# mscaudill/openseize

Hardware: AMD Instinct MI355X
Metric: Msamples/sec/node (FIR+IIR chain, 256ch f64); HBM GB/s vs roofline at 1/2/4/8 GPU (higher is better)
Workload: dtype f64

## Files before the change

openseize_amd/csrc/chain_spec.hip:

```cpp
#include <algorithm>
#include <cmath>
#include <functional>
#include <vector>

#include "common.h"
#include "fft4096.h"
#include "fir_pair.h"
#include "handles.h"
#include "sos_tile.h"
#include "chain_spec.h"
#include "chain_zp.h"

namespace osz {

struct SpecArgs {
    FirArgs f;
    int64_t n;
    int64_t W;
    int nruns;
    int la, lb;
    int R;
    const double *M;
    const double *P;
    const double *Lrow;
// ... 425 lines not shown
    hipLaunchKernelGGL(spec_poison_kernel, dim3((nch + 255) / 256), dim3(256), 0, st, s->dcarry[s->cur],
                       4095 + 256 * s->R, sos->dstate, sos->nsec, nch);
    OSZ_HIP(hipGetLastError());
    s->true_valid = true;
    return OSZ_OK;
}

int spec_touch(ChainSpec *s, hipStream_t st) {
    if (!s) return OSZ_OK;
    int rc = spec_settle(s, st);
    if (rc) return rc;
    s->carry_valid = false;
    return OSZ_OK;
}

using spec_kern_t = void (*)(SpecArgs);
template <int NM, int HP>
static spec_kern_t spec_kernel_for(int nr) {
    static const spec_kern_t k[8] = {
        chain_spec_kernel<8, NM, HP>,  chain_spec_kernel<9, NM, HP>,  chain_spec_kernel<10, NM, HP>,
        chain_spec_kernel<11, NM, HP>, chain_spec_kernel<12, NM, HP>, chain_spec_kernel<13, NM, HP>,
        chain_spec_kernel<14, NM, HP>, chain_spec_kernel<15, NM, HP>};
    return k[nr - 8];
}

static int specn_forward(ChainSpec *s, const double *x, int64_t ldx, int64_t n, double *f, int64_t ldf,
                         hipStream_t st, const std::function<int()> &between, bool *taken) {
    osz_fir_s *fir = s->fir;
    const int NB = s->NR, S = 256 * NB;
    if (n < 2 * (int64_t)S) return OSZ_OK;
    if (!s->carry_valid) {
        int rc = spec_import(s, st);
        if (rc) return rc;
    }
    {
        int rc = between();
        if (rc) return rc;
    }
    const int64_t W = (n - 1) / S;
    int64_t nruns = 512 / fir->nch;
    if (nruns > W) nruns = W;
    if (nruns < 1) nruns = 1;
    ZpArgs g{};
    g.f.x = x;
    g.f.y = f;
    g.f.ldx = ldx;
    g.f.ldy = ldf;
    g.f.n = n;
    g.f.skip = 0;
    g.f.wlen = fir->ntaps;
    g.f.step = S;
    g.f.H = s->dH;
    g.f.tb = fir->tb;
    g.n = n;
    g.W = W;
    g.nruns = (int)nruns;
    g.la = (int)(n - W * S);
    g.R = s->R;
    g.Rf = s->R;
    g.nh = s->nh;
    g.Lrow = s->dT;
    g.carry_in = s->dcarry[s->cur];
    g.carry_out = s->dcarry[s->cur ^ 1];
    if (n >= s->hist_cap) {
        g.hist = s->dhist[s->hcur];
        g.hist_len = s->hist_cap;
        s->hist_n = s->hist_cap;
    } else {
        const int64_t keep = std::min<int64_t>(s->hist_n, s->hist_cap - n);
        double *dst = s->dhist[s->hcur ^ 1];
        if (keep > 0)
            OSZ_HIP(hipMemcpy2DAsync(dst, sizeof(double) * s->hist_cap,
                                     s->dhist[s->hcur] + (s->hist_n - keep), sizeof(double) * s->hist_cap,
                                     sizeof(double) * keep, fir->nch, hipMemcpyDeviceToDevice, st));
        OSZ_HIP(hipMemcpy2DAsync(dst + keep, sizeof(double) * s->hist_cap, x, sizeof(double) * ldx,
                                 sizeof(double) * n, fir->nch, hipMemcpyDeviceToDevice, st));
        s->hcur ^= 1;
        s->hist_n = keep + n;
    }
    s->since_import += n;
    zp_kern_t kern = zpn_fwd_kernel_for(NB, s->NM, s->NS);
    if (!kern) return fail(OSZ_ERR_STATE, "forward chain kernel: no instance for %d rows, %d modes (%d slow)", NB, s->NM, s->NS);
    const int ns = 2 * s->nh;
    const size_t lds = sizeof(fft::cube::C2) * fft::cube::SLOTS +
                       sizeof(double) * (ns + 2 * s->R * s->NS * 2 + s->NM * 2 + 20 * s->NM * 2 + 2 * s->NS * ns) + 1024;
    OSZ_DYN_LDS(kern, lds);
    {
        KernelTimer kt("chain_fwd", st);
        hipLaunchKernelGGL(kern, dim3((unsigned)nruns, fir->nch), dim3(256), lds, st, g);
    }
    OSZ_HIP(hipGetLastError());
    {
        int rcs = sos_seal_launch(g.f.y, g.f.ldy, n, (int)nruns, W, nruns, (int64_t)S, nullptr, 0, fir->nch,
                                  g.carry_out, kSpecLdc, kSpecLdc, st);
        if (rcs) return rcs;
    }
    s->cur ^= 1;
    s->true_valid = false;
    *taken = true;
    return OSZ_OK;
}


static int spec_link(osz_fir_s *fir, osz_sos_s *sos, hipStream_t st, ChainSpec **out) {
    ChainSpec *s = sos->spec;
    if (s && s->fir != fir) {
        int rc = spec_settle(s, st);
        if (rc) return rc;
        spec_unlink(s);
        s = nullptr;
    }
    if (!s && fir->spec) {
        int rc = spec_settle(fir->spec, st);
        if (rc) return rc;
        spec_unlink(fir->spec);
    }
    if (!s) {
        s = new ChainSpec();
        s->fir = fir;
        s->sos = sos;
        fir->spec = sos->spec = s;
        int rc = spec_build(s);
        if (rc) {
            spec_unlink(s);
            return rc;
        }
    }
    *out = s;
    return OSZ_OK;
}

static spec_kern_t spec_kernel_pick(const ChainSpec *s) {
    if (s->NR < 8 || s->NR > 15) return nullptr;
    return s->NM == 2 ? spec_kernel_for<2, 16>(s->NR) : s->NM == 4 ? spec_kernel_for<4, 16>(s->NR)
           : s->NM == 6 ? spec_kernel_for<6, 16>(s->NR) : nullptr;
}

int spec_route(osz_fir_s *fir, osz_sos_s *sos, hipStream_t st, int *route) {
    ChainSpec *s = nullptr;
    int rc = spec_link(fir, sos, st, &s);
    if (rc) return rc;
    *route = !s->eligible ? 0 : s->nega ? 2 : 1;
    return OSZ_OK;
}

int spec_plan(osz_fir_s *fir, osz_sos_s *sos, hipStream_t st, int *route, int *rows, int *nm, int *ns,
              int *has) {
    int rc = spec_route(fir, sos, st, route);
    if (rc || *route == 0) return rc;
    const ChainSpec *s = sos->spec;
    *rows = s->NR;
    *nm = s->NM;
    *ns = s->nega ? s->NS : 0;
    *has = (s->nega ? zpn_fwd_kernel_for(s->NR, s->NM, s->NS) != nullptr : spec_kernel_pick(s) != nullptr);
    return OSZ_OK;
}

int spec_try_forward(osz_fir_s *fir, osz_sos_s *sos, const double *x, int64_t ldx, int64_t n, double *f,
                     int64_t ldf, hipStream_t st, const std::function<int()> &between, bool *taken) {
    *taken = false;
    ChainSpec *s = nullptr;
    {
        int rc = spec_link(fir, sos, st, &s);
        if (rc) return rc;
    }
    if (!s->eligible) return OSZ_OK;
    if (s->nega) return specn_forward(s, x, ldx, n, f, ldf, st, between, taken);
    const int NR = s->NR, S = 256 * NR;
// ... 81 lines not shown
```

openseize_amd/csrc/chain_zp.h:

```cpp
#pragma once

#include "chain_spec.h"
#include "fft4096.h"
#include "fir_pair.h"
#include "handles.h"
#include "nega_window.h"

namespace osz {

struct ZpArgs {
    FirArgs f;
    double *y0;
    int64_t ldy0, n0;
    int64_t n;
    int64_t W;
    int nruns;
    int la, lb;
    int R, Rf, nh;
    const double *M;
    const double *P;
    const double *Lrow;
    const double *carry_in;
    double *carry_out;
    const double *held_in;
    double *held_out;
    double *hist;
    int hist_len;
    long long *nanpos;
    long long pos;
    int wclose;
};

__host__ __device__ __forceinline__ int64_t zp_run_start(int64_t r, int64_t W, int nruns, int wclose) {
    if (r <= 0) return 0;
    if (r >= nruns) return W;
    if (W < 8 * (int64_t)nruns) return (r * W) / nruns;
    const int64_t V = W + (nruns - 1) + wclose;
    const int64_t s = (r * V) / nruns - (r - 1);
    return s < W - (nruns - r) ? s : W - (nruns - r);
}

template <int NM>
__device__ __forceinline__ void zp_powers(const double *ptab, int e, double *pr, double *pi) {
    const double *p1 = ptab + ((e >> 5) * NM) * 2, *p2 = ptab + ((8 + ((e >> 2) & 7)) * NM) * 2,
                 *p3 = ptab + ((16 + (e & 3)) * NM) * 2;
#pragma unroll
    for (int q = 0; q < NM; ++q) {
        const double ar = p1[2 * q] * p2[2 * q] - p1[2 * q + 1] * p2[2 * q + 1];
        const double ai = p1[2 * q] * p2[2 * q + 1] + p1[2 * q + 1] * p2[2 * q];
        pr[q] = ar * p3[2 * q] - ai * p3[2 * q + 1];
        pi[q] = ar * p3[2 * q + 1] + ai * p3[2 * q];
    }
}

template <int NM>
__device__ __forceinline__ double zp_dot(const double *kk, const double *pr, const double *pi) {
    double c = 0.0;
#pragma unroll
    for (int q = 0; q < NM; ++q) c = fma(kk[2 * q], pr[q], fma(-kk[2 * q + 1], pi[q], c));
    return c;
}

__device__ __forceinline__ bool zp_exact_nanpos(const double *xb, int count, int t, long long *nanpos, long long base) {
    int hit = -1;
    for (int i = t; i < count && hit < 0; i += 256)
        if (!(fabs(xb[i]) <= 1.79769313486231570815e308)) hit = i;
    if (hit >= 0) atomicMin(nanpos, base + hit);
    return __syncthreads_or(hit >= 0) != 0;
}

using zp_kern_t = void (*)(ZpArgs);
using spec::zpn_rm_for;
zp_kern_t zpn_kernel_for(int nb, int nm, int ns, int r);
zp_kern_t zpn_fwd_kernel_for(int nb, int nm, int ns);

}
```

openseize_amd/csrc/chain_zp.hip:

```cpp
#include <algorithm>
#include <cmath>
#include <functional>
#include <mutex>
#include <utility>
#include <vector>

#include "chain_zp.h"

namespace osz {

template <int NM, int PER>
__device__ __forceinline__ void zp_fit_kappa_n(int tt, int R, const double *fitbuf, const double *mtab,
                                               const double *lrow, double *kapA, double *kapN) {
    constexpr int ns = 8 * PER;
    if ((tt & ~63) >= 32 * NM) return;
    const int qd = tt >> 3, p8 = tt & 7;
    const bool valid = qd < 4 * NM;
    const int blk = valid ? qd / (2 * NM) : 0, kind = valid ? (qd / NM) % 2 : 0, q = valid ? qd % NM : 0;
    const double *yb = fitbuf + ns * blk + PER * p8;
    const double *mr = mtab + ns * ((2 * kind) * NM + q) + PER * p8;
    const double *mi = mtab + ns * ((2 * kind + 1) * NM + q) + PER * p8;
    constexpr int B = PER % 3 == 0 ? 3 : 4;
    double sr0 = 0.0, sr1 = 0.0, si0 = 0.0, si1 = 0.0;
#pragma unroll
// ... 552 lines not shown
        }
    }
    *out = s;
    return OSZ_OK;
}

template <int NM, bool DMA>
static zp_kern_t zp_kernel_for(int nr) {
    static const zp_kern_t k[8] = {chain_zp_kernel<8, NM, DMA>,  chain_zp_kernel<9, NM, DMA>,
                                   chain_zp_kernel<10, NM, DMA>, chain_zp_kernel<11, NM, DMA>,
                                   chain_zp_kernel<12, NM, DMA>, chain_zp_kernel<13, NM, DMA>,
                                   chain_zp_kernel<14, NM, DMA>, chain_zp_kernel<15, NM, DMA>};
    return k[nr - 8];
}
static zp_kern_t zp_kernel_pick(const ChainZp *s) {
    if (s->nega) return zpn_kernel_for(s->NR, s->NM, s->NS, s->R);
    if (s->NR < 8 || s->NR > 15) return nullptr;
    return s->NM == 2 ? zp_kernel_for<2, true>(s->NR) : s->NM == 4 ? zp_kernel_for<4, true>(s->NR)
           : s->NM == 6 ? zp_kernel_for<6, true>(s->NR) : nullptr;
}
static int zp_launch(ChainZp *s, const double *x, int64_t ldx, int64_t n, double *y0, int64_t ldy0,
                     int64_t n0, double *y, int64_t ldy, hipStream_t st) {
    osz_fir_s *fir = s->fir;
    const int NR = s->NR, S = 256 * NR;
    const int64_t pair = 2 * (int64_t)S;
    const int64_t npw = n / pair, rem = n - npw * pair;
    const int64_t W = s->nega ? (n - 1) / S : rem == 0 ? npw - 1 : npw;
    const int64_t nlast = s->nega ? n - W * S : n - W * pair;
    int64_t nruns = 512 / fir->nch;
    if (nruns > W) nruns = W;
    if (nruns < 1) nruns = 1;
    ZpArgs g{};
    g.f.x = x;
    g.f.y = y;
    g.f.ldx = ldx;
    g.f.ldy = ldy;
    g.f.n = n;
    g.f.skip = 0;
    g.f.wlen = fir->ntaps;
    g.f.step = S;
    g.f.H = s->dH;
    g.f.tb = fir->tb;
    g.y0 = y0;
    g.ldy0 = ldy0;
    g.n0 = n0;
    g.n = n;
    g.W = W;
    g.nruns = (int)nruns;
    g.la = (int)std::min<int64_t>(nlast, S);
    g.lb = (int)(nlast - g.la);
    g.R = s->R;
    g.Rf = s->Rf;
    g.nh = s->nh;
    g.M = s->dM;
    g.P = s->dP;
    g.Lrow = s->dL;
    g.carry_in = s->dcarry[s->cur];
    g.carry_out = s->dcarry[s->cur ^ 1];
    g.held_in = s->dheld[s->cur];
    g.held_out = s->dheld[s->cur ^ 1];
    g.nanpos = s->dnanpos;
    g.pos = s->pos;
    g.wclose = s->nega ? 1 : 4;
    if (n >= s->hist_cap) {
        g.hist = s->dhist[s->hcur];
        g.hist_len = s->hist_cap;
        s->hist_n = s->hist_cap;
    } else {
        const int64_t keep = std::min<int64_t>(s->hist_n, s->hist_cap - n);
        double *dst = s->dhist[s->hcur ^ 1];
        if (keep > 0)
            OSZ_HIP(hipMemcpy2DAsync(dst, sizeof(double) * s->hist_cap, s->dhist[s->hcur] + (s->hist_n - keep),
                                     sizeof(double) * s->hist_cap, sizeof(double) * keep, fir->nch,
                                     hipMemcpyDeviceToDevice, st));
        OSZ_HIP(hipMemcpy2DAsync(dst + keep, sizeof(double) * s->hist_cap, x, sizeof(double) * ldx,
                                 sizeof(double) * n, fir->nch, hipMemcpyDeviceToDevice, st));
        s->hcur ^= 1;
        s->hist_n = keep + n;
        g.hist = nullptr;
        g.hist_len = 0;
    }
    zp_kern_t kern = zp_kernel_pick(s);
    if (!kern) return fail(OSZ_ERR_STATE, "zero-phase kernel: no instance for %d rows, %d modes (%d slow)", NR, s->NM, s->NS);
    const size_t lds = zp_lds_bytes(s);
    OSZ_DYN_LDS(kern, lds);
    {
        KernelTimer kt("chain_zp", st);
        hipLaunchKernelGGL(kern, dim3((unsigned)nruns, fir->nch), dim3(256), lds, st, g);
    }
    OSZ_HIP(hipGetLastError());
    s->cur ^= 1;
    s->pos += n;
    return OSZ_OK;
}

}

using namespace osz;

extern "C" {

int64_t osz_chain_zp_lag(osz_fir_t fir, osz_sos_t sos) {
    if (!fir || !sos) return -1;
    ChainZp *s = nullptr;
    if (zp_get(fir, sos, &s) != OSZ_OK || !s->eligible) return -1;
    return 256 * (int64_t)s->R;
}

int osz_chain_zp_plan(osz_fir_t fir, osz_sos_t sos, int32_t *out, int n) {
    OSZ_REQUIRE(fir && sos && out && n >= 8, "osz_chain_zp_plan: null argument or n=%d < 8", n);
    ChainZp *s = nullptr;
    int rc = zp_get(fir, sos, &s);
    if (rc) return rc;
    for (int i = 0; i < n; ++i) out[i] = 0;
    if (!s->eligible) return OSZ_OK;
    out[0] = s->nega ? 2 : 1;
    out[1] = s->NR;
    out[2] = s->NM;
    out[3] = s->NS;
    out[4] = s->R;
    out[5] = s->Rf;
    out[6] = s->nega ? zpn_rm_for(s->NR, s->R) : kSpecRMax;
    out[7] = zp_kernel_pick(s) != nullptr;
    return OSZ_OK;
}

int osz_chain_zp_tolerance(osz_fir_t fir, osz_sos_t sos, double tol) {
    OSZ_REQUIRE(fir && sos, "osz_chain_zp_tolerance: null handle");
    OSZ_REQUIRE(tol == 0.0 || (tol >= 1e-18 && tol <= 1e-6), "osz_chain_zp_tolerance: tol=%g", tol);
    if (sos->zp && sos->zp->open) return fail(OSZ_ERR_STATE, "osz_chain_zp_tolerance: a zero-phase stream is open");
    if (sos->zp_tol != tol) {
        if (sos->spec) {
            int rc = spec_settle(sos->spec, nullptr);
            if (rc) return rc;
            OSZ_HIP(hipStreamSynchronize(nullptr));
            spec_unlink(sos->spec);
        }
        sos->zp_tol = tol;
        if (sos->zp) zp_unlink(sos->zp);
    }
    return OSZ_OK;
}

int osz_chain_zp_reach(osz_fir_t fir, osz_sos_t sos, int64_t step) {
    OSZ_REQUIRE(fir && sos && step >= 0, "osz_chain_zp_reach: step=%lld", (long long)step);
    ChainZp *s = nullptr;
    int rc = zp_get(fir, sos, &s);
    if (rc) return rc;
    if (!s->eligible)
        return fail(OSZ_ERR_UNSUPPORTED, "osz_chain_zp_reach: this filter pair does not take the zero-phase kernel");
    s->ref_step = step;
    return OSZ_OK;
}

int64_t osz_chain_zp_min_chunk(osz_fir_t fir, osz_sos_t sos) {
    if (!fir || !sos) return -1;
    ChainZp *s = nullptr;
    if (zp_get(fir, sos, &s) != OSZ_OK || !s->eligible) return -1;
    return zp_min_chunk(s);
}

int osz_chain_zp_open(osz_fir_t fir, osz_sos_t sos, int64_t skip, void *stream) {
    OSZ_REQUIRE(fir && sos, "osz_chain_zp_open: null handle");
    OSZ_SAME_DEVICE(fir, "osz_chain_zp_open");
    OSZ_SAME_DEVICE(sos, "osz_chain_zp_open");
    hipStream_t st = as_stream(stream);
    ChainZp *s = nullptr;
// ... 111 lines not shown
```

openseize_amd/csrc/chain_zpn_body.h:

```cpp
#include <type_traits>

#include "chain_zp.h"
#include "nega_window.h"

namespace osz {

template <int NM, int NS, int PER, int RM, bool ZP>
__device__ __forceinline__ void zpn_fit_kappa_n(int tt, int R, const double *fitbuf, const double *mtab,
                                                const double *l256, double *kmu, double *knu) {
    constexpr int ns = 16 * PER;
    constexpr int NA = NS + (ZP ? NM : 0);
    if ((tt & ~63) >= 16 * NA) return;
    const int qd = tt >> 4, p16 = tt & 15;
    const bool valid = qd < NA;
    const bool is_mu = qd < NS;
    const int q = valid ? (is_mu ? qd : qd - NS) : 0;
    const int rre = is_mu ? q : 2 * NS + q, rim = is_mu ? NS + q : 2 * NS + NM + q;
    const double *yb = fitbuf + PER * p16;
    const double *mr = mtab + ns * rre + PER * p16;
    const double *mi = mtab + ns * rim + PER * p16;
    double y[PER], a[PER], b[PER];
#pragma unroll
    for (int k = 0; k < PER; ++k) {
        y[k] = yb[k];
// ... 6 lines not shown
        sr = fma(a[k], y[k], sr);
        si = fma(b[k], y[k], si);
    }
    if (!valid) sr = si = 0.0;
    sr += dpp_row_shr0<1>(sr);
    si += dpp_row_shr0<1>(si);
    sr += dpp_row_shr0<2>(sr);
    si += dpp_row_shr0<2>(si);
    sr += dpp_row_shr0<4>(sr);
    si += dpp_row_shr0<4>(si);
    sr += dpp_row_shr0<8>(sr);
    si += dpp_row_shr0<8>(si);
    if (p16 == 15 && valid) {
        const double lr = l256[q * 2 + 0], li = l256[q * 2 + 1];
        double kr = sr, ki = si;
#pragma unroll
        for (int r = 0; r < RM; ++r) {
            if (r < R) {
                if (is_mu) {
                    kmu[(r * NS + q) * 2 + 0] = kr;
                    kmu[(r * NS + q) * 2 + 1] = ki;
                } else {
                    knu[(r * NM + q) * 2 + 0] = kr;
                    knu[(r * NM + q) * 2 + 1] = ki;
                }
                const double nr = kr * lr - ki * li;
                ki = kr * li + ki * lr;
                kr = nr;
            }
        }
    }
}

template <int NM, int NS, int RM, bool ZP>
__device__ __forceinline__ void zpn_fit_kappa(int tt, int nh, int R, const double *fitbuf, const double *mtab,
                                              const double *l256, double *kmu, double *knu) {
    if (nh == 24) zpn_fit_kappa_n<NM, NS, 3, RM, ZP>(tt, R, fitbuf, mtab, l256, kmu, knu);
    else if (nh == 32) zpn_fit_kappa_n<NM, NS, 4, RM, ZP>(tt, R, fitbuf, mtab, l256, kmu, knu);
    else zpn_fit_kappa_n<NM, NS, 2, RM, ZP>(tt, R, fitbuf, mtab, l256, kmu, knu);
}

template <int NM, int NG>
__device__ __forceinline__ void zpn_powers(const double *ptab, int q0, int e, double *pr, double *pi) {
    const double *p1 = ptab + ((e >> 5) * NM + q0) * 2, *p2 = ptab + ((8 + ((e >> 2) & 7)) * NM + q0) * 2,
                 *p3 = ptab + ((16 + (e & 3)) * NM + q0) * 2;
#pragma unroll
    for (int q = 0; q < NG; ++q) {
        const double ar = p1[2 * q] * p2[2 * q] - p1[2 * q + 1] * p2[2 * q + 1];
        const double ai = p1[2 * q] * p2[2 * q + 1] + p1[2 * q + 1] * p2[2 * q];
        pr[q] = ar * p3[2 * q] - ai * p3[2 * q + 1];
        pi[q] = ar * p3[2 * q + 1] + ai * p3[2 * q];
    }
}

template <int NM>
__device__ __forceinline__ void zpn_dot2(const double *k0, const double *k1, const double *pr, const double *pi,
                                         double &d0, double &d1) {
    double ar = 0.0, ai = 0.0, br = 0.0, bi = 0.0;
#pragma unroll
    for (int q = 0; q < NM; ++q) {
        ar = fma(k0[2 * q], pr[q], ar);
        ai = fma(k0[2 * q + 1], pi[q], ai);
        br = fma(k1[2 * q], pr[q], br);
        bi = fma(k1[2 * q + 1], pi[q], bi);
    }
    d0 = ar - ai;
    d1 = br - bi;
}

template <int D, int NS, int RF>
__device__ __forceinline__ void zpn_fwd_bursts(double *re, const double *kmu, const double *kpm, const double *Pr,
                                               const double *Pi, double &first) {
#pragma unroll
    for (int r = 0; r < RF; ++r) {
        double ca, cp;
        zpn_dot2<NS>(kmu + (r * NS) * 2, kpm + (r * NS) * 2, Pr, Pi, ca, cp);
        re[r] += ca;
        re[D + r] += cp;
        if (r == 0) first = ca;
    }
}

template <int NM, int NS, int RB>
__device__ __forceinline__ void zpn_bwd_bursts(double *im, double *c7, const double *knu, const double *ptab, int e,
                                               const double *Pr, const double *Pi) {
    double nb[RB];
#pragma unroll
    for (int r = 0; r < RB; ++r) nb[r] = zp_dot<NS>(knu + (r * NM) * 2, Pr, Pi);
    if (NM > NS) {
        constexpr int NF = NM > NS ? NM - NS : 1;
        double fr[NF], fi[NF];
        zpn_powers<NM, NF>(ptab, NS, e, fr, fi);
        nb[0] += zp_dot<NF>(knu + NS * 2, fr, fi);
    }
#pragma unroll
    for (int r = 0; r < RB; ++r) {
        im[15 - r] += nb[r];
        c7[r] = nb[r];
    }
}

template <int NB, int NM, int NS, int RM = kSpecRMax, bool ZP = true>
__global__ __launch_bounds__(256, 2) void chain_zpn_kernel(ZpArgs g) {
    constexpr int D = 32 - NB, S = 256 * NB, NHI = NB - 16, NP = (NB + 1) / 2;
    static_assert(NB >= 20 && NB <= 30, "rows per block");
    extern __shared__ fft::cube::C2 cube_lds[];
    const int Rt = g.R;
    const int R = ZP ? g.R : 0;
    const int Rf = g.Rf, nh = g.nh, ns = 2 * nh;
    constexpr int NMROWS = 2 * NS + (ZP ? 2 * NM : 0);
    double *xl = reinterpret_cast<double *>(cube_lds) + 2 * fft::cube::SLOTS;
    double *fitbuf = xl;
    double *kapP = fitbuf + ns;
    double *knu = kapP + 2 * Rt * NS * 2;
    double *lrow = knu + (ZP ? Rt * NM * 2 : 0);
    double *ptab = lrow + NM * 2;
    double *mtab = ptab + 20 * NM * 2;
    fft::cube::C2 *tw2l = reinterpret_cast<fft::cube::C2 *>(mtab + NMROWS * ns);
    const FirArgs &a = g.f;
    const int t = threadIdx.x, run = blockIdx.x, c = blockIdx.y;
    const int L = 256 * R;
    const double *xr = a.x + (int64_t)c * a.ldx;
    const int64_t n = g.n, n0 = g.n0;
    double *y0r = g.y0 ? g.y0 + (int64_t)c * g.ldy0 : nullptr;
    double *yr = a.y + (int64_t)c * a.ldy - n0;
    double *ho = g.held_out + (int64_t)c * L;
    const int p0 = __builtin_amdgcn_readfirstlane(
        (int)(ZP ? zp_run_start(run, g.W, g.nruns, g.wclose) : ((int64_t)run * g.W) / g.nruns));
    const int p1 = __builtin_amdgcn_readfirstlane(
        (int)(ZP ? zp_run_start(run + 1, g.W, g.nruns, g.wclose) : ((int64_t)(run + 1) * g.W) / g.nruns));
    const int first = run == 0 ? 0 : p0 - 1;
    const int lastf = p1 - 1;
    const bool closes = run == g.nruns - 1;

    NegaWindow<NHI> P{a, cube_lds, tw2l};
    {
        fft::cube::TwPow w2;
        fft::nega::tw_load(t, a.tb, P.tw1, w2);
        if (t < 16) {
#pragma unroll
            for (int q = 0; q < 4; ++q) tw2l[16 * q + t] = fft::cube::C2{w2.r[q], w2.i[q]};
        }
    }
    double cr[D];
#pragma unroll
    for (int j = 0; j < D; ++j) cr[j] = 0.0;
    if (first <= lastf) zp_request_rows<NP>(xr + (int64_t)first * S, NB, t, cube_lds);
    {
        const int ntab = NM * 2 + 20 * NM * 2 + NMROWS * ns;
#pragma unroll 8
        for (int i = t; i < ntab; i += 256) lrow[i] = g.Lrow[i];
    }
    for (int i = t; i < 2 * Rt * NS * 2; i += 256) kapP[i] = 0.0;
    double held[RM];
#pragma unroll
    for (int r = 0; r < RM; ++r) held[r] = 0.0;
    bool bad = ZP ? g.nanpos[c] != 0x7fffffffffffffffLL : false;
    int64_t bad_at = 0;
    int par = 0;
    int younger = -1;
    __syncthreads();

#define OSZ_ZP_PUT(i_, v_)                      \
    do {                                        \
        const int64_t q_ = (i_) + L;            \
        if (q_ < n0) y0r[q_] = (v_);            \
        else if (q_ < n) yr[q_] = (v_);         \
        else ho[q_ - n] = (v_);                 \
    } while (0)

    auto block = [&](const int p, auto closing_tag) __attribute__((always_inline)) {
        constexpr bool closing = decltype(closing_tag)::value;
        const int64_t o = (int64_t)p * S;
        double re[16], im[16];
        take_turns();
        if (!closing) {
            if (younger == NB) asm volatile("s_waitcnt vmcnt(%0) ; osz:dma" ::"n"(NB) : "memory");
            else asm volatile("s_waitcnt vmcnt(0) ; osz:dma" ::: "memory");
            int tq = t;
            asm volatile("" : "+v"(tq));
            const double *xs = reinterpret_cast<const double *>(cube_lds) + 128 * (tq >> 6) + (tq & 63);
#pragma unroll
            for (int j = 0; j < 16; ++j) {
                re[j] = xs[512 * (j >> 1) + 64 * (j & 1)];
                im[j] = j < NHI ? xs[512 * ((j + 16) >> 1) + 64 * ((j + 16) & 1)] : 0.0;
            }
        } else {
            const int la = g.la;
            const double *xc = xr + o + t;
#pragma unroll
            for (int j = 0; j < 16; ++j) {
                re[j] = 256 * j + t < la ? xc[256 * j] : 0.0;
                im[j] = (j < NHI && 4096 + 256 * j + t < la) ? xc[4096 + 256 * j] : 0.0;
            }
        }
        P.template transform<NP>(t, re, im, (!closing && p < lastf) ? xr + o + S : nullptr, NB);
        int nst = 0;
        int tt = t;
        asm volatile("" : "+v"(tt));
        const unsigned lane8 = 8u * (unsigned)tt;
        if (tt < nh) fitbuf[tt] = im[15];
        else if (tt >= 256 - nh) fitbuf[tt - 256 + ns] = im[15];
#pragma unroll
        for (int j = 0; j < D; ++j) re[j] += cr[j];
        __syncthreads();
        double *kmu = kapP + (par ^ 1) * (Rt * NS * 2);
        zpn_fit_kappa<NM, NS, RM, ZP>(tt, nh, Rt, fitbuf, mtab, lrow, kmu, knu);
        __syncthreads();
        double c7[RM];
#pragma unroll
        for (int r = 0; r < RM; ++r) c7[r] = 0.0;
        {
            double Pr[NS], Pi[NS];
            zpn_powers<NM, NS>(ptab, 0, tt, Pr, Pi);
            const double *kpm = kapP + par * (Rt * NS * 2);
            double ca = 0.0;
            switch (Rf) {
                case 1: zpn_fwd_bursts<D, NS, 1>(re, kmu, kpm, Pr, Pi, ca); break;
                case 2: zpn_fwd_bursts<D, NS, 2>(re, kmu, kpm, Pr, Pi, ca); break;
                case 3: zpn_fwd_bursts<D, NS, 3>(re, kmu, kpm, Pr, Pi, ca); break;
                case 4: zpn_fwd_bursts<D, NS, 4>(re, kmu, kpm, Pr, Pi, ca); break;
                default: zpn_fwd_bursts<D, NS, 5>(re, kmu, kpm, Pr, Pi, ca); break;
            }
            double Qr[NS], Qi[NS];
            if (ZP) zpn_powers<NM, NS>(ptab, 0, 255 - tt, Qr, Qi);
            if (ZP) switch (R) {
                case 1: zpn_bwd_bursts<NM, NS, 1>(im, c7, knu, ptab, 255 - tt, Qr, Qi); break;
                case 2: zpn_bwd_bursts<NM, NS, 2>(im, c7, knu, ptab, 255 - tt, Qr, Qi); break;
                case 3: zpn_bwd_bursts<NM, NS, 3>(im, c7, knu, ptab, 255 - tt, Qr, Qi); break;
                case 4: zpn_bwd_bursts<NM, NS, 4>(im, c7, knu, ptab, 255 - tt, Qr, Qi); break;
                case 5: zpn_bwd_bursts<NM, NS, 5>(im, c7, knu, ptab, 255 - tt, Qr, Qi); break;
                case 6: zpn_bwd_bursts<NM, NS, RM >= 6 ? 6 : 5>(im, c7, knu, ptab, 255 - tt, Qr, Qi); break;
                case 7: zpn_bwd_bursts<NM, NS, RM >= 7 ? 7 : 5>(im, c7, knu, ptab, 255 - tt, Qr, Qi); break;
                case 8: zpn_bwd_bursts<NM, NS, RM >= 8 ? 8 : 5>(im, c7, knu, ptab, 255 - tt, Qr, Qi); break;
                case 9: zpn_bwd_bursts<NM, NS, RM >= 9 ? 9 : 5>(im, c7, knu, ptab, 255 - tt, Qr, Qi); break;
                case 10: zpn_bwd_bursts<NM, NS, RM >= 10 ? 10 : 5>(im, c7, knu, ptab, 255 - tt, Qr, Qi); break;
                case 11: zpn_bwd_bursts<NM, NS, RM >= 11 ? 11 : 5>(im, c7, knu, ptab, 255 - tt, Qr, Qi); break;
                default: zpn_bwd_bursts<NM, NS, RM >= 12 ? 12 : 5>(im, c7, knu, ptab, 255 - tt, Qr, Qi); break;
            }
            if (!bad && __builtin_amdgcn_readfirstlane((int)sos_not_finite(ca))) {
                bad = true;
                bad_at = o;
                if (ZP && zp_exact_nanpos(xr + o, closing ? g.la : S, tt, reinterpret_cast<long long *>(g.nanpos + c), g.pos + o))
                    bad_at = -1;
            }
        }
        const double qn = spec_qnan();
        const bool own = p >= p0;
        const bool edge = p >= g.W - 1;
        if (run == 0 && p == 0) {
            nst = -1;
            const double *ci = g.carry_in + (int64_t)c * kSpecLdc + tt;
            if (!bad &&
                __builtin_amdgcn_readfirstlane((int)sos_not_finite(g.carry_in[(int64_t)c * kSpecLdc + 4095 + 256 * R]))) {
                bad = true;
                bad_at = 0;
            }
#pragma unroll
            for (int j = 0; j < 16; ++j) {
                re[j] += ci[256 * j];
                if (j < NHI) im[j] += ci[4096 + 256 * j];
            }
            if (ZP) {
                const double *hi = g.held_in + (int64_t)c * L + tt;
#pragma unroll
                for (int r = 0; r < RM; ++r)
                    if (r < R) {
                        const int64_t q = 256 * (R - 1 - r) + tt;
                        (q < n0 ? y0r : yr)[q] = bad ? qn : hi[256 * (R - 1 - r)] + c7[r];
                    }
            }
        } else if (ZP && p > first) {
            if (!bad && !closing && o - S + L >= n0) {
                const __amdgpu_buffer_rsrc_t ry = buf_rsrc(yr + (o - S + L));
#pragma unroll
                for (int r = 0; r < RM; ++r)
                    if (r < R) buf_store(held[r] + c7[r], ry, lane8, 2048u * (NB - 1 - r));
                if (nst >= 0) nst += R;
            } else {
                nst = -1;
                const int64_t ob = o - S + tt;
#pragma unroll
                for (int r = 0; r < RM; ++r)
                    if (r < R) OSZ_ZP_PUT(ob + 256 * (NB - 1 - r), bad ? qn : held[r] + c7[r]);
            }
        }
        if (closing) {
            const int la = g.la;
            double *co = g.carry_out + (int64_t)c * kSpecLdc;
            for (int i = tt; i < kSpecLdc; i += 256) co[i] = bad ? qn : 0.0;
            __syncthreads();
#pragma unroll
            for (int j = 0; j < 32; ++j) {
                const int pp = 256 * j + tt;
                const double v = j < 16 ? re[j & 15] : im[j & 15];
                if (pp < la) OSZ_ZP_PUT(o + pp, bad ? qn : v);
                else if (!bad && pp - la < kSpecLdc) co[pp - la] = v;
            }
            if (!bad) {
                double Pr[NS], Pi[NS];
                zpn_powers<NM, NS>(ptab, 0, tt, Pr, Pi);
                for (int r = 0; r < Rf; ++r) {
                    const int k = 8192 + 256 * r + tt - la;
                    if (k < kSpecLdc) co[k] = zp_dot<NS>(kmu + (r * NS) * 2, Pr, Pi);
                }
            }
            if (g.hist) {
                double *hr = g.hist + (int64_t)c * g.hist_len;
                const double *src = xr + n - g.hist_len;
                for (int i = tt; i < g.hist_len; i += 256) hr[i] = src[i];
            }
        } else {
            if (own) {
                if (!bad && !edge && o + L >= n0) {
                    const __amdgpu_buffer_rsrc_t ry = buf_rsrc(yr + (o + L));
#pragma unroll
                    for (int j = 0; j < 16; ++j) {
                        if (RM <= NHI || j < NB - R) buf_store(re[j], ry, lane8, 2048u * j);
                        if (j < NHI - R) buf_store(im[j], ry, lane8, 2048u * (j + 16));
                    }
                    if (nst >= 0) nst += NB - R;
                } else {
                    nst = -1;
                    int64_t off = o + tt;
                    asm volatile("" : "+v"(off));
#pragma unroll
                    for (int j = 0; j < 16; ++j) {
                        if (RM <= NHI || j < NB - R) OSZ_ZP_PUT(off + 256 * j, bad ? qn : re[j]);
                        if (j < NHI - R) OSZ_ZP_PUT(off + 256 * (j + 16), bad ? qn : im[j]);
                    }
                }
            }
#pragma unroll
            for (int r = 0; r < RM; ++r)
                if (r < R) held[r] = r < NHI ? im[(NHI - 1 - r) & 15] : re[(NB - 1 - r) & 15];
#pragma unroll
            for (int j = 0; j < D; ++j) cr[j] = im[NHI + j];
        }
        par ^= 1;
        younger = nst;
    };
    for (int p = first; p <= lastf; ++p) block(p, std::false_type{});
    if (closes) block(lastf + 1, std::true_type{});
#undef OSZ_ZP_PUT
    if (ZP && bad && bad_at >= 0 && t == 0) atomicMin(reinterpret_cast<long long *>(g.nanpos + c), g.pos + bad_at);
}

template <int NM, int NS>
static zp_kern_t zpn_kernel_nb(int nb, int r) {
    static const zp_kern_t k[7] = {chain_zpn_kernel<24, NM, NS>, chain_zpn_kernel<25, NM, NS>,
                                   chain_zpn_kernel<26, NM, NS>, chain_zpn_kernel<27, NM, NS>,
                                   chain_zpn_kernel<28, NM, NS>, chain_zpn_kernel<29, NM, NS>,
                                   chain_zpn_kernel<30, NM, NS>};
    static const zp_kern_t k8[3] = {chain_zpn_kernel<24, NM, NS, 8>, chain_zpn_kernel<25, NM, NS, 8>,
                                    chain_zpn_kernel<26, NM, NS, 8>};
    static const zp_kern_t k12[4] = {chain_zpn_kernel<20, NM, NS, 12>, chain_zpn_kernel<21, NM, NS, 12>,
                                     chain_zpn_kernel<22, NM, NS, 12>, chain_zpn_kernel<23, NM, NS, 12>};
    switch (zpn_rm_for(nb, r)) {
    case 12: return k12[nb - 20];
    case 8: return k8[nb - 24];
    case kSpecRMax: return k[nb - 24];
    default: return nullptr;
    }
}

#define OSZ_ZPN_CAT2(a, b) a##b
#define OSZ_ZPN_CAT(a, b) OSZ_ZPN_CAT2(a, b)
zp_kern_t OSZ_ZPN_CAT(zpn_kernel_nm, OSZ_ZPN_NM)(int nb, int ns, int r) {
    constexpr int NM = OSZ_ZPN_NM;
    if (nb < 20 || nb > 30) return nullptr;
    if (ns == 2) return zpn_kernel_nb<NM, 2>(nb, r);
    if (NM >= 4 && ns == 4) return zpn_kernel_nb<NM, (NM >= 4 ? 4 : 2)>(nb, r);
    if (NM >= 6 && ns == 6) return zpn_kernel_nb<NM, (NM >= 6 ? 6 : 2)>(nb, r);
    return nullptr;
}

template <int NM, int NS>
static zp_kern_t zpn_fwd_kernel_nb(int nb) {
    static const zp_kern_t k[7] = {
        chain_zpn_kernel<24, NM, NS, kSpecRMax, false>, chain_zpn_kernel<25, NM, NS, kSpecRMax, false>,
        chain_zpn_kernel<26, NM, NS, kSpecRMax, false>, chain_zpn_kernel<27, NM, NS, kSpecRMax, false>,
        chain_zpn_kernel<28, NM, NS, kSpecRMax, false>, chain_zpn_kernel<29, NM, NS, kSpecRMax, false>,
        chain_zpn_kernel<30, NM, NS, kSpecRMax, false>};
    return k[nb - 24];
}
zp_kern_t OSZ_ZPN_CAT(zpn_fwd_kernel_nm, OSZ_ZPN_NM)(int nb, int ns) {
    constexpr int NM = OSZ_ZPN_NM;
    if (nb < 24 || nb > 30) return nullptr;
    if (ns == 2) return zpn_fwd_kernel_nb<NM, 2>(nb);
    if (NM >= 4 && ns == 4) return zpn_fwd_kernel_nb<NM, (NM >= 4 ? 4 : 2)>(nb);
    if (NM >= 6 && ns == 6) return zpn_fwd_kernel_nb<NM, (NM >= 6 ? 6 : 2)>(nb);
    return nullptr;
}

#if OSZ_ZPN_NM == 2
zp_kern_t zpn_fwd_kernel_nm4(int nb, int ns);
zp_kern_t zpn_fwd_kernel_nm6(int nb, int ns);
zp_kern_t zpn_fwd_kernel_nm8(int nb, int ns);
zp_kern_t zpn_fwd_kernel_for(int nb, int nm, int ns) {
    return nm == 2 ? zpn_fwd_kernel_nm2(nb, ns) : nm == 4 ? zpn_fwd_kernel_nm4(nb, ns) : nm == 6 ? zpn_fwd_kernel_nm6(nb, ns)
           : nm == 8 ? zpn_fwd_kernel_nm8(nb, ns) : nullptr;
}
zp_kern_t zpn_kernel_nm4(int nb, int ns, int r);
zp_kern_t zpn_kernel_nm6(int nb, int ns, int r);
zp_kern_t zpn_kernel_nm8(int nb, int ns, int r);
zp_kern_t zpn_kernel_for(int nb, int nm, int ns, int r) {
    return nm == 2 ? zpn_kernel_nm2(nb, ns, r) : nm == 4 ? zpn_kernel_nm4(nb, ns, r) : nm == 6 ? zpn_kernel_nm6(nb, ns, r)
           : nm == 8 ? zpn_kernel_nm8(nb, ns, r) : nullptr;
}
#endif

}
```

openseize_amd/csrc/nega_window.h:

```cpp
#pragma once

#include "common.h"
#include "fft4096.h"
#include "fir_pair.h"

namespace osz {

template <int NP>
__device__ __forceinline__ void zp_request_rows(const double *src, int nrows, int t, const void *cube) {
    int tq = t;
    asm volatile("" : "+v"(tq));
    const __amdgpu_buffer_rsrc_t rx =
        __builtin_amdgcn_make_buffer_rsrc(const_cast<double *>(src), 0, 2048 * nrows, 0x00020000);
    const unsigned voff = 2048u * (((unsigned)tq >> 5) & 1u) + 512u * ((unsigned)tq >> 6) + 16u * ((unsigned)tq & 31u);
    const unsigned ldsb = __builtin_amdgcn_readfirstlane((unsigned)reinterpret_cast<uintptr_t>(cube) +
                                                         1024u * ((unsigned)tq >> 6));
#pragma unroll
    for (int m = 0; m < NP; ++m) {
        unsigned keep;
        asm volatile("s_mov_b32 %0, m0\n\t"
                     "s_mov_b32 m0, %1\n\t"
                     "s_nop 0\n\t"
                     "buffer_load_dwordx4 %2, %3, 0 offen nt lds\n\t"
                     "s_mov_b32 m0, %0"
                     : "=&s"(keep)
                     : "s"(ldsb + 4096u * m), "v"(voff + 4096u * m), "s"(rx)
                     : "memory");
    }
}



template <int NHI>
struct NegaWindow {
    using C2 = fft::cube::C2;
    const FirArgs &a;
    C2 *L;
    const C2 *tw2l;
    fft::nega::TwPowN tw1;

    __device__ __forceinline__ void load_tw2(int t, fft::cube::TwPow &w) const {
        const C2 *p = tw2l + (t & 15);
#pragma unroll
        for (int q = 0; q < 4; ++q) {
            const C2 v = p[16 * q];
            w.r[q] = v.re;
            w.i[q] = v.im;
        }
    }

    template <int NP = 1>
    __device__ __forceinline__ void transform(int t_in, double *re, double *im, const double *next = nullptr,
                                              int nrows = 0) {
        int t = t_in;
        asm volatile("" : "+v"(t));
        fft::nega::f1<NHI>(t, re, im, tw1, L);
        __syncthreads();
        fft::cube::TwPow tw2;
        load_tw2(t, tw2);
        fft::cube2::f2(t, re, im, tw2, L);
        double hr[16], hi[16];
        const unsigned lane16 = 16u * ((unsigned)t & 255u);
        const __amdgpu_buffer_rsrc_t rh = buf_rsrc(a.H);
#pragma unroll
        for (int r = 0; r < 16; ++r) {
            const buf_d2 h = buf_load2(rh, lane16, 4096u * r);
            hr[r] = h.x;
            hi[r] = h.y;
        }
        wave_lds_fence();
        fft::cube2::f3(t, re, im, L);
#pragma unroll
        for (int r = 0; r < 16; ++r) fft::cube::cmul(re[r], im[r], hr[r], hi[r]);
        fft::cube2::i3(t, re, im, L);
        wave_lds_fence();
        load_tw2(t, tw2);
        fft::cube2::i2(t, re, im, tw2, L);
        __syncthreads();
        fft::nega::i1_load(t, re, im, L);
        if (next) {
            asm volatile("s_waitcnt lgkmcnt(0) ; osz:dma" ::: "memory");
            zp_request_rows<NP>(next, nrows, t_in, L);
        }
        fft::nega::i1_finish(re, im, tw1);
    }
};


}
```

Baseline: 253,300.

## Defer kappa fit and burst flush one block to overlap with next FFT

Adds a pipelined mode in the zero-phase/forward chain kernel. The kappa fit for block p is now computed inside the next block's transform, right after the first FFT stage, and its burst corrections are flushed one block later from parked LDS rows. This removes the two per-block barriers around the fit from the critical path. The M table is read from global memory instead of being copied into LDS, which shrinks LDS so the pipe mode can be enabled whenever the footprint stays under 80 KiB. The cost is more complex state (pend/park), a final drain step, extra global reads of the M table, and a risk of correctness bugs in edge and NaN handling.

```diff
diff --git a/openseize_amd/csrc/chain_spec.hip b/openseize_amd/csrc/chain_spec.hip
--- a/openseize_amd/csrc/chain_spec.hip
+++ b/openseize_amd/csrc/chain_spec.hip
@@ -531,8 +531,12 @@
     zp_kern_t kern = zpn_fwd_kernel_for(NB, s->NM, s->NS);
     if (!kern) return fail(OSZ_ERR_STATE, "forward chain kernel: no instance for %d rows, %d modes (%d slow)", NB, s->NM, s->NS);
     const int ns = 2 * s->nh;
-    const size_t lds = sizeof(fft::cube::C2) * fft::cube::SLOTS +
-                       sizeof(double) * (ns + 2 * s->R * s->NS * 2 + s->NM * 2 + 20 * s->NM * 2 + 2 * s->NS * ns) + 1024;
+    const size_t lds_pipe = zpn_pipe_lds_bytes(s->nh, s->NM, s->NS, s->R, 0, s->R, false);
+    g.pipe = lds_pipe <= kZpnPipeLdsMax;
+    const size_t lds = g.pipe ? lds_pipe
+                              : sizeof(fft::cube::C2) * fft::cube::SLOTS +
+                                    sizeof(double) * (ns + 2 * s->R * s->NS * 2 + s->NM * 2 + 20 * s->NM * 2 + 2 * s->NS * ns) +
+                                    1024;
     OSZ_DYN_LDS(kern, lds);
     {
         KernelTimer kt("chain_fwd", st);
diff --git a/openseize_amd/csrc/chain_zp.h b/openseize_amd/csrc/chain_zp.h
--- a/openseize_amd/csrc/chain_zp.h
+++ b/openseize_amd/csrc/chain_zp.h
@@ -29,7 +29,15 @@
     long long *nanpos;
     long long pos;
     int wclose;
+    int pipe;
 };
+
+inline size_t zpn_pipe_lds_bytes(int nh, int NM, int NS, int Rt, int R, int Rf, bool zp) {
+    return sizeof(fft::cube::C2) * fft::cube::SLOTS +
+           sizeof(double) * (2 * nh + 2 * Rt * NS * 2 + (zp ? Rt * NM * 2 : 0) + NM * 2 + 20 * NM * 2 + (R + Rf) * 256) +
+           1024;
+}
+constexpr size_t kZpnPipeLdsMax = 80 * 1024;
 
 __host__ __device__ __forceinline__ int64_t zp_run_start(int64_t r, int64_t W, int nruns, int wclose) {
     if (r <= 0) return 0;
diff --git a/openseize_amd/csrc/chain_zp.hip b/openseize_amd/csrc/chain_zp.hip
--- a/openseize_amd/csrc/chain_zp.hip
+++ b/openseize_amd/csrc/chain_zp.hip
@@ -658,7 +658,9 @@
     }
     zp_kern_t kern = zp_kernel_pick(s);
     if (!kern) return fail(OSZ_ERR_STATE, "zero-phase kernel: no instance for %d rows, %d modes (%d slow)", NR, s->NM, s->NS);
-    const size_t lds = zp_lds_bytes(s);
+    const size_t lds_pipe = s->nega ? zpn_pipe_lds_bytes(s->nh, s->NM, s->NS, s->R, s->R, s->Rf, true) : 0;
+    g.pipe = s->nega && lds_pipe <= kZpnPipeLdsMax;
+    const size_t lds = g.pipe ? lds_pipe : zp_lds_bytes(s);
     OSZ_DYN_LDS(kern, lds);
     {
         KernelTimer kt("chain_zp", st);
diff --git a/openseize_amd/csrc/chain_zpn_body.h b/openseize_amd/csrc/chain_zpn_body.h
--- a/openseize_amd/csrc/chain_zpn_body.h
+++ b/openseize_amd/csrc/chain_zpn_body.h
@@ -112,9 +112,8 @@
 }
 
 template <int NM, int NS, int RB>
-__device__ __forceinline__ void zpn_bwd_bursts(double *im, double *c7, const double *knu, const double *ptab, int e,
-                                               const double *Pr, const double *Pi) {
-    double nb[RB];
+__device__ __forceinline__ void zpn_bwd_amps(double *nb, const double *knu, const double *ptab, int e, const double *Pr,
+                                             const double *Pi) {
 #pragma unroll
     for (int r = 0; r < RB; ++r) nb[r] = zp_dot<NS>(knu + (r * NM) * 2, Pr, Pi);
     if (NM > NS) {
@@ -123,10 +122,34 @@
         zpn_powers<NM, NF>(ptab, NS, e, fr, fi);
         nb[0] += zp_dot<NF>(knu + NS * 2, fr, fi);
     }
+}
+template <int NM, int NS, int RB>
+__device__ __forceinline__ void zpn_bwd_bursts(double *im, double *c7, const double *knu, const double *ptab, int e,
+                                               const double *Pr, const double *Pi) {
+    double nb[RB];
+    zpn_bwd_amps<NM, NS, RB>(nb, knu, ptab, e, Pr, Pi);
 #pragma unroll
     for (int r = 0; r < RB; ++r) {
         im[15 - r] += nb[r];
         c7[r] = nb[r];
+    }
+}
+template <int NM, int NS, int RM>
+__device__ __forceinline__ void zpn_bwd_amps_r(int R, double *nb, const double *knu, const double *ptab, int e,
+                                               const double *Pr, const double *Pi) {
+    switch (R) {
+        case 1: zpn_bwd_amps<NM, NS, 1>(nb, knu, ptab, e, Pr, Pi); break;
+        case 2: zpn_bwd_amps<NM, NS, 2>(nb, knu, ptab, e, Pr, Pi); break;
+        case 3: zpn_bwd_amps<NM, NS, 3>(nb, knu, ptab, e, Pr, Pi); break;
+        case 4: zpn_bwd_amps<NM, NS, 4>(nb, knu, ptab, e, Pr, Pi); break;
+        case 5: zpn_bwd_amps<NM, NS, 5>(nb, knu, ptab, e, Pr, Pi); break;
+        case 6: zpn_bwd_amps<NM, NS, RM >= 6 ? 6 : 5>(nb, knu, ptab, e, Pr, Pi); break;
+        case 7: zpn_bwd_amps<NM, NS, RM >= 7 ? 7 : 5>(nb, knu, ptab, e, Pr, Pi); break;
+        case 8: zpn_bwd_amps<NM, NS, RM >= 8 ? 8 : 5>(nb, knu, ptab, e, Pr, Pi); break;
+        case 9: zpn_bwd_amps<NM, NS, RM >= 9 ? 9 : 5>(nb, knu, ptab, e, Pr, Pi); break;
+        case 10: zpn_bwd_amps<NM, NS, RM >= 10 ? 10 : 5>(nb, knu, ptab, e, Pr, Pi); break;
+        case 11: zpn_bwd_amps<NM, NS, RM >= 11 ? 11 : 5>(nb, knu, ptab, e, Pr, Pi); break;
+        default: zpn_bwd_amps<NM, NS, RM >= 12 ? 12 : 5>(nb, knu, ptab, e, Pr, Pi); break;
     }
 }
 
@@ -138,6 +161,7 @@
     const int Rt = g.R;
     const int R = ZP ? g.R : 0;
     const int Rf = g.Rf, nh = g.nh, ns = 2 * nh;
+    const bool pipe = g.pipe != 0;
     constexpr int NMROWS = 2 * NS + (ZP ? 2 * NM : 0);
     double *xl = reinterpret_cast<double *>(cube_lds) + 2 * fft::cube::SLOTS;
     double *fitbuf = xl;
@@ -146,7 +170,9 @@
     double *lrow = knu + (ZP ? Rt * NM * 2 : 0);
     double *ptab = lrow + NM * 2;
     double *mtab = ptab + 20 * NM * 2;
-    fft::cube::C2 *tw2l = reinterpret_cast<fft::cube::C2 *>(mtab + NMROWS * ns);
+    double *park = mtab;
+    const double *mglob = g.Lrow + NM * 2 + 20 * NM * 2;
+    fft::cube::C2 *tw2l = reinterpret_cast<fft::cube::C2 *>(mtab + (pipe ? (R + Rf) * 256 : NMROWS * ns));
     const FirArgs &a = g.f;
     const int t = threadIdx.x, run = blockIdx.x, c = blockIdx.y;
     const int L = 256 * R;
@@ -177,7 +203,7 @@
     for (int j = 0; j < D; ++j) cr[j] = 0.0;
     if (first <= lastf) zp_request_rows<NP>(xr + (int64_t)first * S, NB, t, cube_lds);
     {
-        const int ntab = NM * 2 + 20 * NM * 2 + NMROWS * ns;
+        const int ntab = NM * 2 + 20 * NM * 2 + (pipe ? 0 : NMROWS * ns);
 #pragma unroll 8
         for (int i = t; i < ntab; i += 256) lrow[i] = g.Lrow[i];
     }
@@ -189,6 +215,7 @@
     int64_t bad_at = 0;
     int par = 0;
     int younger = -1;
+    int pend = -1;
     __syncthreads();
 
 #define OSZ_ZP_PUT(i_, v_)                      \
@@ -198,6 +225,77 @@
         else if (q_ < n) yr[q_] = (v_);         \
         else ho[q_ - n] = (v_);                 \
     } while (0)
+
+    auto flush = [&](const int tt, double *cmu, double *cnu) __attribute__((always_inline)) -> int {
+        const int pb = pend;
+        const int64_t ob = (int64_t)pb * S;
+        const bool opening = run == 0 && pb == 0;
+        const unsigned lane8 = 8u * (unsigned)tt;
+        const double qn = spec_qnan();
+        int nst = 0;
+        {
+            double Pr[NS], Pi[NS];
+            zpn_powers<NM, NS>(ptab, 0, tt, Pr, Pi);
+            const bool own = pb >= p0;
+            const bool fast = !bad && pb < g.W - 1 && ob + L >= n0;
+            const __amdgpu_buffer_rsrc_t ry = buf_rsrc(yr + (ob + L));
+            const double *ci = g.carry_in + (int64_t)c * kSpecLdc + tt;
+#pragma unroll
+            for (int r = 0; r < kSpecRMax; ++r)
+                if (r < Rf) {
+                    const double *k = kapP + (r * NS) * 2;
+                    double ar = 0.0, ai = 0.0;
+#pragma unroll
+                    for (int q = 0; q < NS; ++q) {
+                        ar = fma(k[2 * q], Pr[q], ar);
+                        ai = fma(k[2 * q + 1], Pi[q], ai);
+                    }
+                    const double ca = ar - ai;
+                    cmu[r] = ca;
+                    if (own) {
+                        double v = park[(R + r) * 256 + tt] + ca;
+                        if (opening) v += ci[256 * r];
+                        if (fast) buf_store(v, ry, lane8, 2048u * r);
+                        else OSZ_ZP_PUT(ob + tt + 256 * r, bad ? qn : v);
+                    }
+                }
+            if (own) nst = fast ? Rf : -1;
+        }
+        if (ZP) {
+            double Qr[NS], Qi[NS], c7[RM];
+            zpn_powers<NM, NS>(ptab, 0, 255 - tt, Qr, Qi);
+#pragma unroll
+            for (int r = 0; r < RM; ++r) c7[r] = 0.0;
+            zpn_bwd_amps_r<NM, NS, RM>(R, c7, knu, ptab, 255 - tt, Qr, Qi);
+#pragma unroll
+            for (int r = 0; r < RM; ++r) cnu[r] = c7[r];
+            if (opening) {
+                nst = -1;
+                const double *hi = g.held_in + (int64_t)c * L + tt;
+#pragma unroll
+                for (int r = 0; r < RM; ++r)
+                    if (r < R) {
+                        const int64_t q = 256 * (R - 1 - r) + tt;
+                        (q < n0 ? y0r : yr)[q] = bad ? qn : hi[256 * (R - 1 - r)] + c7[r];
+                    }
+            } else if (pb > first) {
+                if (!bad && ob - S + L >= n0) {
+                    const __amdgpu_buffer_rsrc_t rh = buf_rsrc(yr + (ob - S + L));
+#pragma unroll
+                    for (int r = 0; r < RM; ++r)
+                        if (r < R) buf_store(park[r * 256 + tt] + c7[r], rh, lane8, 2048u * (NB - 1 - r));
+                    if (nst >= 0) nst += R;
+                } else {
+                    nst = -1;
+                    const int64_t oh = ob - S + tt;
+#pragma unroll
+                    for (int r = 0; r < RM; ++r)
+                        if (r < R) OSZ_ZP_PUT(oh + 256 * (NB - 1 - r), bad ? qn : park[r * 256 + tt] + c7[r]);
+                }
+            }
+        }
+        return nst;
+    };
 
     auto block = [&](const int p, auto closing_tag) __attribute__((always_inline)) {
         constexpr bool closing = decltype(closing_tag)::value;
@@ -224,18 +322,101 @@
                 im[j] = (j < NHI && 4096 + 256 * j + t < la) ? xc[4096 + 256 * j] : 0.0;
             }
         }
-        P.template transform<NP>(t, re, im, (!closing && p < lastf) ? xr + o + S : nullptr, NB);
+        P.template transform<NP>(t, re, im, (!closing && p < lastf) ? xr + o + S : nullptr, NB,
+                                 [&]() __attribute__((always_inline)) {
+                                     if (pipe && pend >= 0) {
+                                         int tf = t;
+                                         asm volatile("" : "+v"(tf));
+                                         zpn_fit_kappa<NM, NS, RM, ZP>(tf, nh, Rt, fitbuf, mglob, lrow, kapP, knu);
+                                     }
+                                 });
         int nst = 0;
         int tt = t;
         asm volatile("" : "+v"(tt));
         const unsigned lane8 = 8u * (unsigned)tt;
         if (tt < nh) fitbuf[tt] = im[15];
         else if (tt >= 256 - nh) fitbuf[tt - 256 + ns] = im[15];
+        if (pipe) {
+            if (pend >= 0) {
+                double cmu[kSpecRMax], cnu[RM];
+                nst = flush(tt, cmu, cnu);
+#pragma unroll
+                for (int r = 0; r < kSpecRMax; ++r)
+                    if (r < Rf && D + r < 16) re[D + r] += cmu[r];
+#pragma unroll
+                for (int r = 0; r < RM; ++r)
+                    if (r < D && r < R) cr[D - 1 - r] += cnu[r];
+            } else {
+#pragma unroll
+                for (int r = 0; r < kSpecRMax; ++r)
+                    if (r < Rf && D + r < 16) re[D + r] += 0.0;
+            }
+        }
 #pragma unroll
         for (int j = 0; j < D; ++j) re[j] += cr[j];
+        const double qn = spec_qnan();
+        const bool own = p >= p0;
+        const bool edge = p >= g.W - 1;
+        if (pipe && !closing) {
+            if (!bad && __builtin_amdgcn_readfirstlane((int)sos_not_finite(im[15]))) {
+                bad = true;
+                bad_at = o;
+                if (ZP && zp_exact_nanpos(xr + o, S, tt, reinterpret_cast<long long *>(g.nanpos + c), g.pos + o))
+                    bad_at = -1;
+            }
+            if (run == 0 && p == 0) {
+                nst = -1;
+                const double *ci = g.carry_in + (int64_t)c * kSpecLdc + tt;
+                if (!bad &&
+                    __builtin_amdgcn_readfirstlane((int)sos_not_finite(g.carry_in[(int64_t)c * kSpecLdc + 4095 + 256 * R]))) {
+                    bad = true;
+                    bad_at = 0;
+                }
+#pragma unroll
+                for (int j = 0; j < 16; ++j) {
+                    if (j >= Rf) re[j] += ci[256 * j];
+                    if (j < NHI) im[j] += ci[4096 + 256 * j];
+                }
+            }
+            if (own) {
+                if (!bad && !edge && o + L >= n0) {
+                    const __amdgpu_buffer_rsrc_t ry = buf_rsrc(yr + (o + L));
+#pragma unroll
+                    for (int j = 0; j < 16; ++j) {
+                        if (j >= Rf && (RM <= NHI || j < NB - R)) buf_store(re[j], ry, lane8, 2048u * j);
+                        if (j < NHI - R) buf_store(im[j], ry, lane8, 2048u * (j + 16));
+                    }
+                    if (nst >= 0) nst += NB - R - Rf;
+                } else {
+                    nst = -1;
+                    int64_t off = o + tt;
+                    asm volatile("" : "+v"(off));
+#pragma unroll
+                    for (int j = 0; j < 16; ++j) {
+                        if (j >= Rf && (RM <= NHI || j < NB - R)) OSZ_ZP_PUT(off + 256 * j, bad ? qn : re[j]);
+                        if (j < NHI - R) OSZ_ZP_PUT(off + 256 * (j + 16), bad ? qn : im[j]);
+                    }
+                }
+            }
+#pragma unroll
+            for (int r = 0; r < RM; ++r)
+                if (r < R) park[r * 256 + tt] = held[r];
+#pragma unroll
+            for (int r = 0; r < kSpecRMax; ++r)
+                if (r < Rf) park[(R + r) * 256 + tt] = re[r];
+#pragma unroll
+            for (int r = 0; r < RM; ++r)
+                if (r < R) held[r] = r < NHI ? im[(NHI - 1 - r) & 15] : re[(NB - 1 - r) & 15];
+#pragma unroll
+            for (int j = 0; j < D; ++j) cr[j] = im[NHI + j];
+            pend = p;
+            younger = nst;
+            return;
+        }
         __syncthreads();
-        double *kmu = kapP + (par ^ 1) * (Rt * NS * 2);
-        zpn_fit_kappa<NM, NS, RM, ZP>(tt, nh, Rt, fitbuf, mtab, lrow, kmu, knu);
+        double *kmu = pipe ? kapP : kapP + (par ^ 1) * (Rt * NS * 2);
+        if (pipe) zpn_fit_kappa<NM, NS, RM, ZP>(tt, nh, Rt, fitbuf, mglob, lrow, kmu, knu);
+        else zpn_fit_kappa<NM, NS, RM, ZP>(tt, nh, Rt, fitbuf, mtab, lrow, kmu, knu);
         __syncthreads();
         double c7[RM];
 #pragma unroll
@@ -243,7 +424,7 @@
         {
             double Pr[NS], Pi[NS];
             zpn_powers<NM, NS>(ptab, 0, tt, Pr, Pi);
-            const double *kpm = kapP + par * (Rt * NS * 2);
+            const double *kpm = kapP + (pipe ? 1 : par) * (Rt * NS * 2);
             double ca = 0.0;
             switch (Rf) {
                 case 1: zpn_fwd_bursts<D, NS, 1>(re, kmu, kpm, Pr, Pi, ca); break;
@@ -275,9 +456,6 @@
                     bad_at = -1;
             }
         }
-        const double qn = spec_qnan();
-        const bool own = p >= p0;
-        const bool edge = p >= g.W - 1;
         if (run == 0 && p == 0) {
             nst = -1;
             const double *ci = g.carry_in + (int64_t)c * kSpecLdc + tt;
@@ -371,6 +549,15 @@
         younger = nst;
     };
     for (int p = first; p <= lastf; ++p) block(p, std::false_type{});
+    if (pipe && pend >= 0 && !closes) {
+        int tt = t;
+        asm volatile("" : "+v"(tt));
+        __syncthreads();
+        zpn_fit_kappa<NM, NS, RM, ZP>(tt, nh, Rt, fitbuf, mglob, lrow, kapP, knu);
+        __syncthreads();
+        double cmu[kSpecRMax], cnu[RM];
+        (void)flush(tt, cmu, cnu);
+    }
     if (closes) block(lastf + 1, std::true_type{});
 #undef OSZ_ZP_PUT
     if (ZP && bad && bad_at >= 0 && t == 0) atomicMin(reinterpret_cast<long long *>(g.nanpos + c), g.pos + bad_at);
diff --git a/openseize_amd/csrc/nega_window.h b/openseize_amd/csrc/nega_window.h
--- a/openseize_amd/csrc/nega_window.h
+++ b/openseize_amd/csrc/nega_window.h
@@ -31,6 +31,10 @@
 
 
 
+struct NoHook {
+    __device__ __forceinline__ void operator()() const {}
+};
+
 template <int NHI>
 struct NegaWindow {
     using C2 = fft::cube::C2;
@@ -49,13 +53,14 @@
         }
     }
 
-    template <int NP = 1>
+    template <int NP = 1, class AfterF1 = NoHook>
     __device__ __forceinline__ void transform(int t_in, double *re, double *im, const double *next = nullptr,
-                                              int nrows = 0) {
+                                              int nrows = 0, AfterF1 after_f1 = AfterF1{}) {
         int t = t_in;
         asm volatile("" : "+v"(t));
         fft::nega::f1<NHI>(t, re, im, tw1, L);
         __syncthreads();
+        after_f1();
         fft::cube::TwPow tw2;
         load_tw2(t, tw2);
         fft::cube2::f2(t, re, im, tw2, L);
```

After: 244,900 (median of 2 runs). 3.3% lower.
